# weidafeng/Efficient-SlowFast

Measured on AMD Instinct MI355X. Metric: clips/sec (8x8 224^2 SlowFast-R50+CMDA, train step fwd+bwd+allreduce+SGD), higher is better.
Workload: dtype f32

## Files before the change

### efficient-slowfast_amd/csrc/conv_bx.hip

```cpp
#include "bx.h"
#include <stdlib.h>

namespace {

constexpr int BXC_BM = 256;
constexpr int BXC_BK = 16;
constexpr int BXC_STAGES = 3;
constexpr int BXC_ROWB = BXC_BK * 2;
constexpr int BXC_A_STAGE = 3 * BXC_BM * BXC_ROWB;

struct BxArgs {
  sf_conv_desc d;
  const unsigned short* ap;
  const unsigned short* bp;
  float* ws;
  const float* scale;
  const float* bias;
  const float* res;
  float* out;
  int M, ntaps, cpk, nk, S, nk_per, nb_n, tiles;
  int tap_major;
  unsigned a_rows, a_bytes, b_bytes;
  unsigned a_plane, b_plane;
  unsigned wo_mul, wo_sh, ho_mul, ho_sh, to_mul, to_sh;
// ... 146 lines not shown
      cur_aso = (unsigned)l.c * (unsigned)BXC_ROWB;
    }
    const unsigned cur_bso = (unsigned)(l.tap * p.cpk + l.c) * (unsigned)BXC_ROWB;
    if constexpr (AF32) {
      __builtin_amdgcn_raw_ptr_buffer_load_lds(x_rs, (lds_void*)(smem + stage * STAGE + wave * 2048), 16, cur_f0, cur_aso,
                                               0, 0);
      __builtin_amdgcn_raw_ptr_buffer_load_lds(x_rs, (lds_void*)(smem + stage * STAGE + wave * 2048 + 1024), 16, cur_f1,
                                               cur_aso, 0, 0);
    } else {
      char* const sa = smem + stage * STAGE + wave * 1024;
#pragma unroll
      for (int g = 0; g < 3; ++g)
        __builtin_amdgcn_raw_ptr_buffer_load_lds(a_rs, (lds_void*)(sa + g * (BXC_BM * BXC_ROWB)), 16, cur_voff,
                                                 cur_aso + (unsigned)g * p.a_plane, 0, 0);
    }
    if (b_loader) {
      char* const sb = smem + stage * STAGE + A_ST + wave * 1024;
#pragma unroll
      for (int g = 0; g < 3; ++g)
        __builtin_amdgcn_raw_ptr_buffer_load_lds(b_rs, (lds_void*)(sb + g * (BN * BXC_ROWB)), 16, b_voff,
                                                 cur_bso + (unsigned)g * p.b_plane, 0, 0);
    }
    ls = next(l);
  };

  const unsigned frag_lane = (unsigned)(lane & 31) * BXC_ROWB + (unsigned)(((lane >> 5) ^ ((lane >> 4) & 1)) * 16);
  const unsigned a_frag = (unsigned)(wm * 64) * BXC_ROWB + frag_lane;
  const unsigned b_frag = A_ST + (unsigned)(wn * (BN / 2)) * BXC_ROWB + frag_lane;
  unsigned f_frag[2][2] = {{0, 0}, {0, 0}};
  if constexpr (AF32) {
#pragma unroll
    for (int i = 0; i < 2; ++i) {
      const int r = wm * 64 + i * 32 + (lane & 31);
#pragma unroll
      for (int q = 0; q < 2; ++q) f_frag[i][q] = (unsigned)r * 64u + (unsigned)(((2 * (lane >> 5) + q) ^ ((r >> 2) & 3)) * 16);
    }
  }

  f32x16 acc[2][NT];
#pragma unroll
  for (int i = 0; i < 2; ++i)
#pragma unroll
    for (int j = 0; j < NT; ++j)
#pragma unroll
      for (int e = 0; e < 16; ++e) acc[i][j][e] = 0.f;

  if (nsteps > 0) issue(0);
  if (nsteps > 1) issue(1);
  for (int it = 0; it < nsteps; ++it) {
    if (it + 1 < nsteps) {
      if constexpr (AF32) {
        if (b_loader) asm volatile("s_waitcnt vmcnt(5)" ::: "memory");
        else asm volatile("s_waitcnt vmcnt(2)" ::: "memory");
      } else {
        if (b_loader) asm volatile("s_waitcnt vmcnt(6)" ::: "memory");
        else asm volatile("s_waitcnt vmcnt(3)" ::: "memory");
      }
    } else {
      asm volatile("s_waitcnt vmcnt(0)" ::: "memory");
    }
    __builtin_amdgcn_s_barrier();
    if (it + 2 < nsteps) issue((it + 2) % BXC_STAGES);
    const char* const st = smem + (it % BXC_STAGES) * STAGE;
    u32x4 af[2][3], bf[NT][3];
    if constexpr (AF32) {
#pragma unroll
      for (int i = 0; i < 2; ++i) {
        const f32x4 lo = *reinterpret_cast<const f32x4*>(st + f_frag[i][0]);
        const f32x4 hi = *reinterpret_cast<const f32x4*>(st + f_frag[i][1]);
        split_pair(lo[0], lo[1], af[i], 0);
        split_pair(lo[2], lo[3], af[i], 1);
        split_pair(hi[0], hi[1], af[i], 2);
        split_pair(hi[2], hi[3], af[i], 3);
      }
    }
#pragma unroll
    for (int pc = 0; pc < 3; ++pc) {
      if constexpr (!AF32) {
#pragma unroll
        for (int i = 0; i < 2; ++i)
          af[i][pc] = *reinterpret_cast<const u32x4*>(st + a_frag + pc * (BXC_BM * BXC_ROWB) + i * (32 * BXC_ROWB));
      }
#pragma unroll
      for (int j = 0; j < NT; ++j)
        bf[j][pc] = *reinterpret_cast<const u32x4*>(st + b_frag + pc * (BN * BXC_ROWB) + j * (32 * BXC_ROWB));
    }
#pragma unroll
    for (int i = 0; i < 2; ++i)
#pragma unroll
      for (int j = 0; j < NT; ++j) acc[i][j] = mfma_split(af[i], bf[j], acc[i][j]);
  }

  const int col = lane & 31, rsub = 4 * (lane >> 5);
  if (DIRECT) {
#pragma unroll
    for (int j = 0; j < NT; ++j) {
      const int n = n0 + wn * (BN / 2) + j * 32 + col;
      const bool n_ok = n < d.Cout;
      const float sc = (p.scale && n_ok) ? p.scale[n] : 1.f;
      const float bi = (p.bias && n_ok) ? p.bias[n] : 0.f;
#pragma unroll
      for (int i = 0; i < 2; ++i) {
        float r[16];
#pragma unroll
        for (int e = 0; e < 16; ++e) {
          const int m = m0 + wm * 64 + i * 32 + (e & 3) + 8 * (e >> 2) + rsub;
          r[e] = (p.res && m < p.M && n_ok) ? p.res[(long)m * d.res_cs + d.res_coff + n] : 0.f;
        }
#pragma unroll
        for (int e = 0; e < 16; ++e) {
          const int m = m0 + wm * 64 + i * 32 + (e & 3) + 8 * (e >> 2) + rsub;
          if (m < p.M && n_ok) p.out[(long)m * d.out_cs + d.out_coff + n] = sf_act(acc[i][j][e] * sc + bi + r[e], d.act);
        }
      }
    }
    return;
  }
  float* const wsp = p.ws + (long)split * p.M * d.Cout;
#pragma unroll
  for (int i = 0; i < 2; ++i)
#pragma unroll
    for (int j = 0; j < NT; ++j) {
      const int n = n0 + wn * (BN / 2) + j * 32 + col;
#pragma unroll
      for (int e = 0; e < 16; ++e) {
        const int m = m0 + wm * 64 + i * 32 + (e & 3) + 8 * (e >> 2) + rsub;
        if (m < p.M && n < d.Cout) wsp[(long)m * d.Cout + n] = acc[i][j][e];
      }
    }
}

template <int BN>
__global__ __launch_bounds__(512, 4) void conv_pw_bx_kernel(const BxArgs p) {
  constexpr int A_STAGE = BXC_BM * 64;
  constexpr int B_STAGE = 3 * BN * BXC_ROWB;
  constexpr int STAGE = A_STAGE + B_STAGE;
  constexpr int NT = BN / 64;
  extern __shared__ __attribute__((aligned(16))) char smem[];
  const sf_conv_desc& d = p.d;
  const int tid = threadIdx.x, lane = tid & 63;
  const int wave = __builtin_amdgcn_readfirstlane(tid >> 6);
  const int wm = wave & 3, wn = wave >> 2;
  const int bid = xcd_remap(blockIdx.x, p.tiles);
  const int tile_m = bid / p.nb_n, tile_n = bid - tile_m * p.nb_n;
  const int m0 = tile_m * BXC_BM, n0 = tile_n * BN;
  const int nsteps = p.nk;

  const int lrow = lane >> 1;
  const unsigned lchunk = (unsigned)((lane & 1) ^ ((lrow >> 4) & 1)) * 16u;
  const bool b_loader = BN == 256 || wave < BN / 32;
  const int bn = n0 + 32 * wave + lrow;
  const unsigned kbytes = (unsigned)p.nk * (unsigned)BXC_ROWB;
  const unsigned b_voff = (unsigned)((b_loader && bn < d.Cout) ? bn : d.Cout) * kbytes + lchunk;
  const __amdgpu_buffer_rsrc_t b_rs = __builtin_amdgcn_make_buffer_rsrc((void*)p.bp, 0, p.b_bytes, 0x00020000);
  const __amdgpu_buffer_rsrc_t x_rs = __builtin_amdgcn_make_buffer_rsrc((void*)p.xf, 0, p.xf_bytes, 0x00020000);
  unsigned a_lvoff[2];
#pragma unroll
  for (int u = 0; u < 2; ++u) {
    const int r = 32 * wave + 16 * u + (lane >> 2);
    const int m = m0 + r;
    const unsigned chunk = (unsigned)((lane & 3) ^ ((r >> 2) & 3));
    a_lvoff[u] = m < p.M ? ((unsigned)m * (unsigned)d.in_cs + (unsigned)d.in_coff) * 4u + chunk * 16u : 0x80000000u;
  }
  auto issue = [&](int step) {
    char* const st = smem + (step % 2) * STAGE;
#pragma unroll
    for (int u = 0; u < 2; ++u)
      __builtin_amdgcn_raw_ptr_buffer_load_lds(x_rs, (lds_void*)(st + wave * 2048 + u * 1024), 16, a_lvoff[u],
                                               (unsigned)step * 64u, 0, 0);
    if (b_loader) {
      char* const sb = st + A_STAGE + wave * 1024;
#pragma unroll
      for (int g = 0; g < 3; ++g)
        __builtin_amdgcn_raw_ptr_buffer_load_lds(b_rs, (lds_void*)(sb + g * (BN * BXC_ROWB)), 16, b_voff,
                                                 (unsigned)step * (unsigned)BXC_ROWB + (unsigned)g * p.b_plane, 0, 0);
    }
  };
  unsigned a_frag[2][2];
#pragma unroll
  for (int i = 0; i < 2; ++i) {
    const int r = wm * 64 + i * 32 + (lane & 31);
#pragma unroll
    for (int q = 0; q < 2; ++q)
      a_frag[i][q] = (unsigned)r * 64u + (unsigned)(((2 * (lane >> 5) + q) ^ ((r >> 2) & 3)) * 16);
  }
  const unsigned frag_lane = (unsigned)(lane & 31) * BXC_ROWB + (unsigned)(((lane >> 5) ^ ((lane >> 4) & 1)) * 16);
  const unsigned b_frag = A_STAGE + (unsigned)(wn * (BN / 2)) * BXC_ROWB + frag_lane;

  f32x16 acc[2][NT];
#pragma unroll
  for (int i = 0; i < 2; ++i)
#pragma unroll
    for (int j = 0; j < NT; ++j)
#pragma unroll
      for (int e = 0; e < 16; ++e) acc[i][j][e] = 0.f;

  if (nsteps > 0) issue(0);
  for (int it = 0; it < nsteps; ++it) {
    asm volatile("s_waitcnt vmcnt(0)" ::: "memory");
    __builtin_amdgcn_s_barrier();
    if (it + 1 < nsteps) issue(it + 1);
    const char* const st = smem + (it % 2) * STAGE;
    u32x4 af[2][3], bf[NT][3];
#pragma unroll
    for (int i = 0; i < 2; ++i) {
      const f32x4 lo = *reinterpret_cast<const f32x4*>(st + a_frag[i][0]);
      const f32x4 hi = *reinterpret_cast<const f32x4*>(st + a_frag[i][1]);
      split_pair(lo[0], lo[1], af[i], 0);
      split_pair(lo[2], lo[3], af[i], 1);
      split_pair(hi[0], hi[1], af[i], 2);
      split_pair(hi[2], hi[3], af[i], 3);
    }
#pragma unroll
    for (int pc = 0; pc < 3; ++pc)
#pragma unroll
      for (int j = 0; j < NT; ++j)
        bf[j][pc] = *reinterpret_cast<const u32x4*>(st + b_frag + pc * (BN * BXC_ROWB) + j * (32 * BXC_ROWB));
#pragma unroll
    for (int i = 0; i < 2; ++i)
#pragma unroll
      for (int j = 0; j < NT; ++j) acc[i][j] = mfma_split(af[i], bf[j], acc[i][j]);
  }

  const int col = lane & 31, rsub = 4 * (lane >> 5);
  const bool want_stats = p.stats != nullptr;
  float* const kred = reinterpret_cast<float*>(smem);
  if (want_stats) __syncthreads();
#pragma unroll
  for (int j = 0; j < NT; ++j) {
    const int cl = wn * (BN / 2) + j * 32 + col;
    const int n = n0 + cl;
    const bool n_ok = n < d.Cout;
    const float sc = (p.scale && n_ok) ? p.scale[n] : 1.f;
    const float bi = (p.bias && n_ok) ? p.bias[n] : 0.f;
#pragma unroll
    for (int i = 0; i < 2; ++i) {
      float r[16];
#pragma unroll
      for (int e = 0; e < 16; ++e) {
        const int m = m0 + wm * 64 + i * 32 + (e & 3) + 8 * (e >> 2) + rsub;
        r[e] = (p.res && m < p.M && n_ok) ? p.res[(long)m * d.res_cs + d.res_coff + n] : 0.f;
      }
#pragma unroll
      for (int e = 0; e < 16; ++e) {
        const int m = m0 + wm * 64 + i * 32 + (e & 3) + 8 * (e >> 2) + rsub;
        const float v = sf_act(acc[i][j][e] * sc + bi + r[e], d.act);
        acc[i][j][e] = v;
        if (m < p.M && n_ok) p.out[(long)m * d.out_cs + d.out_coff + n] = v;
      }
    }
    if (want_stats && wm == 0 && rsub == 0) kred[cl] = acc[0][j][0];
  }
  if (!want_stats) return;
  __syncthreads();
  float* const sred = kred + BN;
#pragma unroll
  for (int j = 0; j < NT; ++j) {
    const int cl = wn * (BN / 2) + j * 32 + col;
    const float k0 = kred[cl];
    float s1 = 0.f, s2 = 0.f;
#pragma unroll
    for (int i = 0; i < 2; ++i)
#pragma unroll
      for (int e = 0; e < 16; ++e) {
        const int m = m0 + wm * 64 + i * 32 + (e & 3) + 8 * (e >> 2) + rsub;
        if (m < p.M) {
          const float dv = acc[i][j][e] - k0;
          s1 += dv;
          s2 += dv * dv;
        }
      }
    s1 += __shfl_xor(s1, 32, 64);
    s2 += __shfl_xor(s2, 32, 64);
    if (rsub == 0) {
      sred[(wm * BN + cl) * 2] = s1;
      sred[(wm * BN + cl) * 2 + 1] = s2;
    }
  }
  __syncthreads();
  if (tid < BN) {
    const int n = n0 + tid;
    if (n < d.Cout) {
      float s1 = 0.f, s2 = 0.f;
#pragma unroll
      for (int w = 0; w < 4; ++w) {
        s1 += sred[(w * BN + tid) * 2];
        s2 += sred[(w * BN + tid) * 2 + 1];
      }
      const int left = p.M - m0;
      const float cnt = (float)(left < BXC_BM ? left : BXC_BM);
      float* const o = p.stats + ((long)tile_m * (d.Cout >> 2) + (n >> 2)) * 16 + (n & 3);
      o[0] = cnt;
      o[4] = kred[tid];
      o[8] = s1;
      o[12] = s2;
    }
  }
}

struct BxwArgs {
  sf_conv_desc d;
  const unsigned short* xp;
  const unsigned short* zp;
  float* part;
  int M, Kc, S, chunk, nb_col, tiles;
  unsigned x_rows, x_plane, x_bytes, z_plane, z_bytes;
  unsigned wo_mul, wo_sh, ho_mul, ho_sh, to_mul, to_sh, ci_mul, ci_sh;
};

__device__ __forceinline__ u32x2 lds_tr(const char* p) {
  return lds_read_tr(reinterpret_cast<const unsigned short*>(p));
}
__device__ __forceinline__ u32x2 lds_tr_raw(unsigned lds_byte_addr) {
  u32x2 r;
  asm volatile("ds_read_b64_tr_b16 %0, %1" : "=v"(r) : "v"(lds_byte_addr));
  return r;
}

template <int BCO>
__global__ __launch_bounds__(512, 2) void conv_bx_wgrad_kernel(const BxwArgs p) {
  constexpr int BCOL = 256;
  constexpr int NWC = BCO == 256 ? 2 : 4;
  constexpr int NT = BCOL / NWC / 32;
  constexpr int ROW_A = BCO * 2, ROW_B = BCOL * 2;
  constexpr int PL_A = 16 * ROW_A, PL_B = 16 * ROW_B;
  constexpr int A_STAGE = 3 * PL_A, STAGE = A_STAGE + 3 * PL_B;
  constexpr int NA = PL_A / 1024;
  constexpr int CPR_A = BCO / 8;
  extern __shared__ __attribute__((aligned(16))) char smem[];
  const sf_conv_desc& d = p.d;
  const int tid = threadIdx.x, lane = tid & 63;
  const int wave = __builtin_amdgcn_readfirstlane(tid >> 6);
  const int wr = wave / NWC, wc = wave - wr * NWC;
  const int bid = xcd_remap(blockIdx.x, p.tiles * p.S);
  const int split = bid / p.tiles, tile = bid - split * p.tiles;
  const int tile_co = tile / p.nb_col, tile_col = tile - tile_co * p.nb_col;
  const int co0 = tile_co * BCO, col0 = tile_col * BCOL;
  const int mb = split * p.chunk;
  const int me = mb + p.chunk < p.M ? mb + p.chunk : p.M;
  const int nsteps = me > mb ? (me - mb + 15) / 16 : 0;

  const int b_pos = 2 * wave + (lane >> 5);
  const int b_cs = (lane & 31) ^ ((b_pos & 3) << 2);
  const int b_col = col0 + b_cs * 8;
  const bool b_colok = b_col < p.Kc;
  const unsigned b_tap = b_colok ? mdiv((unsigned)b_col, p.ci_mul, p.ci_sh) : 0u;
  const unsigned b_ci = b_colok ? (unsigned)b_col - b_tap * (unsigned)d.Cin : 0u;
  const int b_kw = (int)(b_tap % (unsigned)d.kW), b_kh = (int)((b_tap / (unsigned)d.kW) % (unsigned)d.kH),
            b_kt = (int)(b_tap / (unsigned)(d.kW * d.kH));
  const int b_dt = b_kt * d.dT - d.pT, b_dh = b_kh * d.dH - d.pH, b_dw = b_kw * d.dW - d.pW;
  const unsigned x_rowb = (unsigned)d.Cin * 2u;
  auto b_voff = [&](int m) -> unsigned {
    unsigned r = p.x_rows;
    if (m < me && b_colok) {
      const unsigned q1 = mdiv((unsigned)m, p.wo_mul, p.wo_sh);
      const int wo = (int)((unsigned)m - q1 * (unsigned)d.Wo);
      const unsigned q2 = mdiv(q1, p.ho_mul, p.ho_sh);
      const int ho = (int)(q1 - q2 * (unsigned)d.Ho);
      const unsigned q3 = mdiv(q2, p.to_mul, p.to_sh);
      const int to = (int)(q2 - q3 * (unsigned)d.To);
      const int ti = to * d.sT + b_dt, hi = ho * d.sH + b_dh, wi = wo * d.sW + b_dw;
      if ((unsigned)ti < (unsigned)d.Ti && (unsigned)hi < (unsigned)d.Hi && (unsigned)wi < (unsigned)d.Wi)
        r = (unsigned)((((int)q3 * d.Ti + ti) * d.Hi + hi) * d.Wi + wi);
    }
    return r * x_rowb + b_ci * 2u;
  };
  const bool a_loader = wave < NA;
  const int a_pos = wave * (64 / CPR_A) + lane / CPR_A;
  const int a_cs = (lane % CPR_A) ^ ((a_pos & 3) << 2);
  const int a_co = co0 + a_cs * 8;
  const unsigned z_rowb = (unsigned)d.Cout * 2u;
  auto a_voff = [&](int m) -> unsigned {
    const unsigned r = (m < me && a_co < d.Cout) ? (unsigned)m : (unsigned)p.M;
    return r * z_rowb + (unsigned)(a_co < d.Cout ? a_co : 0) * 2u;
  };
  const __amdgpu_buffer_rsrc_t x_rs = __builtin_amdgcn_make_buffer_rsrc((void*)p.xp, 0, p.x_bytes, 0x00020000);
  const __amdgpu_buffer_rsrc_t z_rs = __builtin_amdgcn_make_buffer_rsrc((void*)p.zp, 0, p.z_bytes, 0x00020000);
  int l_m = mb;
  auto issue = [&](int stage) {
    char* const st = smem + stage * STAGE;
    if (a_loader) {
      const unsigned vo = a_voff(l_m + a_pos);
#pragma unroll
      for (int pc = 0; pc < 3; ++pc)
        __builtin_amdgcn_raw_ptr_buffer_load_lds(z_rs, (lds_void*)(st + pc * PL_A + wave * 1024), 16, vo,
                                                 (unsigned)pc * p.z_plane, 0, 0);
    }
    const unsigned vb = b_voff(l_m + b_pos);
#pragma unroll
    for (int pc = 0; pc < 3; ++pc)
      __builtin_amdgcn_raw_ptr_buffer_load_lds(x_rs, (lds_void*)(st + A_STAGE + pc * PL_B + wave * 1024), 16, vb,
                                               (unsigned)pc * p.x_plane, 0, 0);
    l_m += 16;
  };

  const int g = lane >> 4, q = (lane & 15) >> 2, pq = lane & 3, h = g >> 1;
  unsigned a_addr[2], b_addr[NT];
#pragma unroll
  for (int i = 0; i < 2; ++i) {
    const int ch = wr * 64 + i * 32 + 16 * (g & 1) + 4 * pq;
    a_addr[i] = (unsigned)((8 * h + q) * ROW_A + (((ch >> 3) ^ (q << 2)) << 4) + (ch & 7) * 2);
  }
#pragma unroll
  for (int j = 0; j < NT; ++j) {
    const int ch = wc * (BCOL / NWC) + j * 32 + 16 * (g & 1) + 4 * pq;
    b_addr[j] = (unsigned)(A_STAGE + (8 * h + q) * ROW_B + (((ch >> 3) ^ (q << 2)) << 4) + (ch & 7) * 2);
  }

  f32x16 acc[2][NT];
#pragma unroll
  for (int i = 0; i < 2; ++i)
#pragma unroll
    for (int j = 0; j < NT; ++j)
#pragma unroll
      for (int e = 0; e < 16; ++e) acc[i][j][e] = 0.f;
  const unsigned lds_base = (unsigned)(uintptr_t)(__attribute__((address_space(3))) char*)smem;

  if (nsteps > 0) issue(0);
  if (nsteps > 1) issue(1);
  for (int it = 0; it < nsteps; ++it) {
    if (it + 1 < nsteps) {
      if (a_loader) asm volatile("s_waitcnt vmcnt(6)" ::: "memory");
      else asm volatile("s_waitcnt vmcnt(3)" ::: "memory");
    } else {
      asm volatile("s_waitcnt vmcnt(0)" ::: "memory");
    }
    __builtin_amdgcn_s_barrier();
    const unsigned st = lds_base + (unsigned)((it % BXC_STAGES) * STAGE);
    u32x4 af[2][3], bf[NT][3];
#pragma unroll
    for (int pc = 0; pc < 3; ++pc) {
#pragma unroll
      for (int i = 0; i < 2; ++i) {
        const u32x2 lo = lds_tr_raw(st + a_addr[i] + pc * PL_A), hi = lds_tr_raw(st + a_addr[i] + pc * PL_A + 4 * ROW_A);
        af[i][pc] = (u32x4){lo[0], lo[1], hi[0], hi[1]};
      }
#pragma unroll
      for (int j = 0; j < NT; ++j) {
        const u32x2 lo = lds_tr_raw(st + b_addr[j] + pc * PL_B), hi = lds_tr_raw(st + b_addr[j] + pc * PL_B + 4 * ROW_B);
        bf[j][pc] = (u32x4){lo[0], lo[1], hi[0], hi[1]};
      }
    }
    __builtin_amdgcn_sched_barrier(0);
    if (it + 2 < nsteps) issue((it + 2) % BXC_STAGES);
    __builtin_amdgcn_sched_barrier(0);
#pragma unroll
    for (int pc = 0; pc < 3; ++pc) {
      if constexpr (NT == 4)
        asm volatile("s_waitcnt lgkmcnt(0)"
                     : "+v"(af[0][pc]), "+v"(af[1][pc]), "+v"(bf[0][pc]), "+v"(bf[1][pc]), "+v"(bf[2][pc]), "+v"(bf[3][pc]));
      else
        asm volatile("s_waitcnt lgkmcnt(0)" : "+v"(af[0][pc]), "+v"(af[1][pc]), "+v"(bf[0][pc]), "+v"(bf[1][pc]));
    }
#pragma unroll
    for (int i = 0; i < 2; ++i)
#pragma unroll
      for (int j = 0; j < NT; ++j) acc[i][j] = mfma_split(af[i], bf[j], acc[i][j]);
  }

  float* const out = p.part + (long)split * d.Cout * p.Kc;
  const int ccol = lane & 31, rsub = 4 * (lane >> 5);
#pragma unroll
  for (int i = 0; i < 2; ++i)
#pragma unroll
    for (int j = 0; j < NT; ++j) {
      const int col = col0 + wc * (BCOL / NWC) + j * 32 + ccol;
#pragma unroll
      for (int e = 0; e < 16; ++e) {
        const int co = co0 + wr * 64 + i * 32 + (e & 3) + 8 * (e >> 2) + rsub;
        if (co < d.Cout && col < p.Kc) out[(long)co * p.Kc + col] = acc[i][j][e];
      }
    }
}

__global__ __launch_bounds__(256) void bx_split_rows_kernel(const float* __restrict__ x, int cs, int coff, long rows,
                                                            int C, unsigned short* __restrict__ planes) {
  const int c8 = C >> 3;
  const long total = (rows + 1) * c8;
  const long plane = (rows + 1) * (long)C;
  for (long idx = (long)blockIdx.x * 256 + threadIdx.x; idx < total; idx += (long)gridDim.x * 256) {
    const long r = idx / c8;
    const int c = (int)(idx - r * c8) * 8;
    u32x4 w[3];
    if (r < rows) {
      const f32x4 v0 = *reinterpret_cast<const f32x4*>(x + r * cs + coff + c);
      const f32x4 v1 = *reinterpret_cast<const f32x4*>(x + r * cs + coff + c + 4);
      split_pair(v0[0], v0[1], w, 0);
      split_pair(v0[2], v0[3], w, 1);
      split_pair(v1[0], v1[1], w, 2);
      split_pair(v1[2], v1[3], w, 3);
    } else {
      w[0] = w[1] = w[2] = (u32x4){0u, 0u, 0u, 0u};
    }
#pragma unroll
    for (int pc = 0; pc < 3; ++pc) *reinterpret_cast<u32x4*>(planes + pc * plane + r * C + c) = w[pc];
  }
}

struct BxSplitItem {
  const float* x;
  unsigned short* planes;
  long rows;
  int C, pad_;
};
__global__ __launch_bounds__(256) void bx_split_batched_kernel(const BxSplitItem* __restrict__ items,
                                                               const int* __restrict__ blk0, int n) {
  int lo = 0, hi = n;
  while (hi - lo > 1) {
    const int mid = (lo + hi) >> 1;
    if (blk0[mid] <= (int)blockIdx.x) lo = mid; else hi = mid;
  }
  const BxSplitItem it = items[lo];
  const int c8 = it.C >> 3;
  const long idx = (long)((int)blockIdx.x - blk0[lo]) * 256 + threadIdx.x;
  if (idx >= (it.rows + 1) * c8) return;
  const long plane = (it.rows + 1) * (long)it.C;
  const long r = idx / c8;
  const int c = (int)(idx - r * c8) * 8;
  u32x4 w[3];
  if (r < it.rows) {
    const f32x4 v0 = *reinterpret_cast<const f32x4*>(it.x + r * it.C + c);
    const f32x4 v1 = *reinterpret_cast<const f32x4*>(it.x + r * it.C + c + 4);
    split_pair(v0[0], v0[1], w, 0);
    split_pair(v0[2], v0[3], w, 1);
    split_pair(v1[0], v1[1], w, 2);
    split_pair(v1[2], v1[3], w, 3);
  } else {
    w[0] = w[1] = w[2] = (u32x4){0u, 0u, 0u, 0u};
  }
#pragma unroll
  for (int pc = 0; pc < 3; ++pc) *reinterpret_cast<u32x4*>(it.planes + pc * plane + r * it.C + c) = w[pc];
}

void magic(unsigned dv, unsigned* mul, unsigned* sh) {
  if (dv <= 1) { *mul = 0; *sh = 0; return; }
  unsigned l = 0;
  while ((1u << l) < dv) ++l;
  const unsigned long long num = 1ull << (31 + l);
  *mul = (unsigned)((num + dv - 1) / dv);
  *sh = l - 1;
}

int g_bx_enable = 1;

struct BxPlan { int bn, S, nk, nk_per, nb_n, tiles, direct; long a_rows; };

bool bx_af32(const sf_conv_desc* d);

bool bx_plan(const sf_conv_desc* d, BxPlan* pl, bool gate = true) {
  if (!g_bx_enable) return false;
  const long M = (long)d->N * d->To * d->Ho * d->Wo;
  const int ntaps = d->kT * d->kH * d->kW;
  if ((d->Cin % 16) || d->cin_pad != d->Cin || (d->in_cs % 4) || (d->in_coff % 4)) return false;
  if (d->Cout < 128 || (d->Cout % 4) || d->out_cmul != 1) return false;
  const int nk = ntaps * (d->Cin / BXC_BK);
  if (nk < 32 || M < 2048 || M > 0x7fffffffL) return false;
  if (d->transposed && (d->sT != 1 || d->sH != 1 || d->sW != 1)) return false;
  const long a_rows = (long)d->N * d->Ti * d->Hi * d->Wi;
  if (3 * (a_rows + 1) * d->Cin * 2 > 0xfffffff0L) return false;
  if (3L * (d->Cout + 1) * nk * BXC_ROWB > 0xfffffff0L) return false;
  pl->bn = d->Cout >= 256 ? 256 : 128;
  pl->nb_n = sf_cdiv(d->Cout, pl->bn);
  pl->tiles = sf_cdiv(M, BXC_BM) * pl->nb_n;
  pl->nk = nk;
  pl->a_rows = a_rows;
  const bool scatter = d->os_T > 1 || d->os_H > 1 || d->os_W > 1;
  const double step_us = pl->bn == 256 ? 2.05 : 1.6;
  const double out_mb = (double)M * d->Cout * 4e-6;
  int best = 1;
  double best_t = 1e30;
  for (int S = 1; S <= 16 && nk / S >= 8; ++S) {
    const long wg = (long)pl->tiles * S;
    if (wg > 2048) break;
    const long rounds = sf_cdiv(wg, 256);
    double t = 6.0 + (double)rounds * sf_cdiv(nk, S) * step_us;
    if (S > 1 || scatter) t += 3.0 + out_mb * (2.0 * S + 1.0) / 4.0;
    else t += out_mb / 4.0;
    if (t < best_t - 1e-9) { best_t = t; best = S; }
  }
  pl->S = best;
  pl->nk_per = sf_cdiv(nk, best);
  pl->direct = (best == 1 && !scatter) ? 1 : 0;
  if (gate && g_bx_enable < 2) {
    const double flop = 2.0 * M * (double)nk * BXC_BK * d->Cout;
    const double wave_us = flop / (nk >= 64 ? 100e6 : 90e6);
    const double split_us = bx_af32(d) ? 0.0 : 4.0 + (double)a_rows * d->Cin * 10e-6 / 3.0;
    const double pad = (double)(pl->nb_n * pl->bn) / (double)d->Cout;
    if (best_t * pad + split_us > 0.93 * wave_us) return false;
  }
  return true;
}


int g_pw_enable = 1;

struct PwPlan { int bn, nb_n, tiles, nk; };

bool pw_plan(const sf_conv_desc* d, PwPlan* pl, bool gate = true) {
  if (!g_bx_enable || !g_pw_enable) return false;
  if (d->kT != 1 || d->kH != 1 || d->kW != 1 || d->sT != 1 || d->sH != 1 || d->sW != 1 || d->pT || d->pH || d->pW)
    return false;
  if (d->To != d->Ti || d->Ho != d->Hi || d->Wo != d->Wi) return false;
  if (d->os_T > 1 || d->os_H > 1 || d->os_W > 1 || d->out_cmul != 1) return false;
  if ((d->Cin % 16) || d->cin_pad != d->Cin || (d->in_cs % 4) || (d->in_coff % 4)) return false;
  if (d->Cin < 64 || d->Cout < 64 || (d->Cout % 4)) return false;
  const long M = (long)d->N * d->To * d->Ho * d->Wo;
  if (M < 2048 || M > 0x3fffffffL) return false;
  if (((M - 1) * d->in_cs + d->in_coff + d->Cin) * 4L >= 0x7fffffffL) return false;
  pl->nk = d->Cin / BXC_BK;
  if (3L * (d->Cout + 1) * pl->nk * BXC_ROWB > 0xfffffff0L) return false;
  pl->bn = d->Cout <= 64 ? 64 : 128;
  pl->nb_n = sf_cdiv(d->Cout, pl->bn);
  pl->tiles = sf_cdiv(M, BXC_BM) * pl->nb_n;
  if (gate && g_pw_enable < 2 && g_bx_enable < 2) {
    const double mb = (double)M * (d->Cin + d->Cout) * 4e-6;
    if (pl->bn == 64) {
      if (d->Cin < 128) return false;
      return true;
    }
    if (d->Cout < 128) return false;
    double t_pw = 6.0 + (double)sf_cdiv(pl->tiles, 256) * pl->nk * 1.5;
    if (t_pw < mb / 4.5) t_pw = mb / 4.5;
    const double t_f32 = 6.0 + 2.0 * M * (double)d->Cin * d->Cout / 95e6 + 0.5 * mb / 4.5;
    if (t_pw > 0.85 * t_f32) return false;
  }
  return true;
}

template <int BN>
int launch_pw(const BxArgs& a, int grid, hipStream_t stream) {
  constexpr int lds = 2 * (BXC_BM * 64 + 3 * BN * BXC_ROWB);
  static_assert(lds >= (BN + 4 * BN * 2) * 4, "the statistics scratch lives in the stages");
  static SfLdsAttr at;
  if (!sf_ensure_dyn_lds(at, reinterpret_cast<const void*>(conv_pw_bx_kernel<BN>), lds)) return SF_ELAUNCH;
  hipLaunchKernelGGL((conv_pw_bx_kernel<BN>), dim3(grid), dim3(512), lds, stream, a);
  SF_CHECK_LAUNCH();
  return SF_OK;
}

bool bx_af32(const sf_conv_desc* d) {
  const long rows = (long)d->N * d->Ti * d->Hi * d->Wi;
  return ((rows - 1) * d->in_cs + d->in_coff + d->Cin) * 4L < 0x7fffffffL;
}

long align4(long floats) { return (floats + 3) & ~3L; }
long a_plane_floats(const sf_conv_desc* d, long a_rows) { return align4((3 * (a_rows + 1) * d->Cin + 1) / 2); }
long b_plane_floats(const sf_conv_desc* d, int nk) { return align4((3L * (d->Cout + 1) * nk * BXC_BK + 1) / 2); }

template <int BN, bool DIRECT, bool AF32>
int launch_bx_v(const BxArgs& a, int grid, hipStream_t stream) {
  constexpr int lds = BXC_STAGES * ((AF32 ? BXC_BM * 64 : BXC_A_STAGE) + 3 * BN * BXC_ROWB);
  static SfLdsAttr at;
  if (!sf_ensure_dyn_lds(at, reinterpret_cast<const void*>(conv_bx_kernel<BN, DIRECT, AF32>), lds)) return SF_ELAUNCH;
  hipLaunchKernelGGL((conv_bx_kernel<BN, DIRECT, AF32>), dim3(grid), dim3(512), lds, stream, a);
  SF_CHECK_LAUNCH();
  return SF_OK;
}

template <int BN, bool DIRECT>
int launch_bx(const BxArgs& a, int grid, hipStream_t stream) {
  if (a.xf) return launch_bx_v<BN, DIRECT, true>(a, grid, stream);
  return launch_bx_v<BN, DIRECT, false>(a, grid, stream);
}

}

int sf_conv_bx_tune(int value) { g_bx_enable = value; return SF_OK; }

int sf_conv_bx_takes(const sf_conv_desc* d) {
  BxPlan pl;
  return bx_plan(d, &pl) ? 1 : 0;
}

extern "C" long sf_bx_planes_elems(long rows, int C) { return 3 * (rows + 1) * (long)C; }

int sf_bx_split_rows(const float* x, int cs, int coff, long rows, int C, unsigned short* planes, hipStream_t s) {
  if ((C & 7) || (cs & 3) || (coff & 3) || !sf_aligned16(x) || !sf_aligned16(planes)) return SF_EALIGN;
  const long total = (rows + 1) * (C >> 3);
  long blocks = (total + 255) / 256;
  if (blocks > 256 * 16) blocks = 256 * 16;
  hipLaunchKernelGGL(bx_split_rows_kernel, dim3((unsigned)blocks), dim3(256), 0, s, x, cs, coff, rows, C, planes);
  SF_CHECK_LAUNCH();
  return SF_OK;
}

extern "C" int sf_bx_split(const float* x, int cs, int coff, long rows, int C, unsigned short* planes, void* stream) {
  if (!x || !planes || rows <= 0 || C <= 0) return SF_EINVAL;
  return sf_bx_split_rows(x, cs, coff, rows, C, planes, (hipStream_t)stream);
}

extern "C" int sf_bx_split_batched(const void* items, const int* blk0, int n, int nblocks, void* stream) {
  if (!items || !blk0 || n <= 0 || nblocks <= 0) return SF_EINVAL;
  hipLaunchKernelGGL(bx_split_batched_kernel, dim3(nblocks), dim3(256), 0, (hipStream_t)stream,
                     reinterpret_cast<const BxSplitItem*>(items), blk0, n);
  SF_CHECK_LAUNCH();
  return SF_OK;
}

int sf_conv_pw_tune(int value) { g_pw_enable = value; return SF_OK; }

int sf_conv_pw_takes(const sf_conv_desc* d) {
  PwPlan pl;
  return pw_plan(d, &pl) ? 1 : 0;
}

extern "C" long sf_conv_pw_ws_floats(const sf_conv_desc* d, int have_w_planes) {
  PwPlan pl;
  if (!d || !pw_plan(d, &pl)) return 0;
  return 4 + (have_w_planes ? 0 : b_plane_floats(d, pl.nk));
}

extern "C" long sf_conv_pw_stats_floats(const sf_conv_desc* d) {
  PwPlan pl;
  if (!d || d->transposed || d->act != SF_ACT_NONE || !pw_plan(d, &pl)) return 0;
  const long M = (long)d->N * d->To * d->Ho * d->Wo;
  return (long)sf_cdiv(M, BXC_BM) * 4 * d->Cout;
}

int sf_conv_pw_try(const sf_conv_desc* d, const float* in, const float* w_packed, const unsigned short* w_planes,
                   const float* scale, const float* bias, const float* res, float* out, float* ws, float* stats,
                   int* parts, hipStream_t stream) {
  PwPlan pl;
  if (parts) *parts = 0;
  if (!ws || !pw_plan(d, &pl)) return 1;
  if (!sf_aligned16(in) || !sf_aligned16(w_packed) || !sf_aligned16(ws)) return 1;
  if (w_planes && !sf_aligned16(w_planes)) return SF_EALIGN;
  if (stats && (scale || res || d->act != SF_ACT_NONE || !parts || !sf_aligned16(stats))) return 1;
  const long M = (long)d->N * d->To * d->Ho * d->Wo;
  if (!w_planes) {
    unsigned short* const bp = reinterpret_cast<unsigned short*>(ws + 4);
    const int rc = sf_bx_split_rows(w_packed, pl.nk * BXC_BK, 0, d->Cout, pl.nk * BXC_BK, bp, stream);
    if (rc != SF_OK) return rc;
    w_planes = bp;
  }
  BxArgs a = {};
  a.d = *d;
  a.bp = w_planes;
  a.scale = scale; a.bias = bias; a.res = res; a.out = out;
  a.M = (int)M;
  a.ntaps = 1; a.cpk = pl.nk; a.nk = pl.nk; a.S = 1; a.nk_per = pl.nk; a.nb_n = pl.nb_n; a.tiles = pl.tiles;
  a.b_plane = (unsigned)((long)(d->Cout + 1) * pl.nk * BXC_ROWB);
  a.b_bytes = 3u * a.b_plane;
  a.xf = in;
  a.xf_bytes = (unsigned)(((M - 1) * d->in_cs + d->in_coff + d->Cin) * 4L);
  a.stats = stats;
  if (stats) *parts = (int)sf_cdiv(M, BXC_BM);
  if (pl.bn == 64) return launch_pw<64>(a, pl.tiles, stream);
  return launch_pw<128>(a, pl.tiles, stream);
}

extern "C" int sf_conv_fwd_pw(const sf_conv_desc* d, const float* in, const float* w_packed,
                              const unsigned short* w_planes, const float* scale, const float* bias, const float* res,
                              float* out, float* ws, float* stats, int* parts, void* stream) {
  if (!d || !in || !w_packed || !out || !ws) return SF_EINVAL;
  const int rc = sf_conv_pw_try(d, in, w_packed, w_planes, scale, bias, res, out, ws, stats, parts, (hipStream_t)stream);
  return rc == 1 ? SF_ENOTTAKEN : rc;
}

extern "C" long sf_conv_bx_ws_floats(const sf_conv_desc* d, int have_in_planes, int have_w_planes) {
  BxPlan pl;
  if (!d || !bx_plan(d, &pl)) return 0;
  const long M = (long)d->N * d->To * d->Ho * d->Wo;
  return 4 + ((have_in_planes || bx_af32(d)) ? 0 : a_plane_floats(d, pl.a_rows)) +
         (have_w_planes ? 0 : b_plane_floats(d, pl.nk)) + (pl.direct ? 0 : (long)pl.S * M * d->Cout);
}

int sf_conv_splitk_finish(const sf_conv_desc* d, const float* ws, int S, const float* scale, const float* bias,
                          const float* res, float* out, hipStream_t s);

int sf_conv_bx_try(const sf_conv_desc* d, const float* in, const unsigned short* in_planes, const float* w_packed,
                   const unsigned short* w_planes, const float* scale, const float* bias, const float* res, float* out,
                   float* ws, hipStream_t stream) {
  BxPlan pl;
  if (!ws || !bx_plan(d, &pl)) return 1;
  if (!sf_aligned16(in) || !sf_aligned16(w_packed) || !sf_aligned16(ws)) return 1;
  if ((in_planes && !sf_aligned16(in_planes)) || (w_planes && !sf_aligned16(w_planes))) return SF_EALIGN;
  const long M = (long)d->N * d->To * d->Ho * d->Wo;
  float* cur = ws;
  int rc = SF_OK;
  const bool af32 = bx_af32(d);
  if (!in_planes && !af32) {
    unsigned short* const ap = reinterpret_cast<unsigned short*>(cur);
    cur += a_plane_floats(d, pl.a_rows);
    rc = sf_bx_split_rows(in, d->in_cs, d->in_coff, pl.a_rows, d->Cin, ap, stream);
    if (rc != SF_OK) return rc;
    in_planes = ap;
  }
  if (!w_planes) {
    unsigned short* const bp = reinterpret_cast<unsigned short*>(cur);
    cur += b_plane_floats(d, pl.nk);
    rc = sf_bx_split_rows(w_packed, pl.nk * BXC_BK, 0, d->Cout, pl.nk * BXC_BK, bp, stream);
    if (rc != SF_OK) return rc;
    w_planes = bp;
  }
  BxArgs a = {};
  a.d = *d;
  a.ap = in_planes; a.bp = w_planes; a.ws = cur;
  if (af32) {
    a.xf = in;
    a.xf_bytes = (unsigned)(((pl.a_rows - 1) * d->in_cs + d->in_coff + d->Cin) * 4L);
  }
  a.scale = scale; a.bias = bias; a.res = res; a.out = out;
  a.M = (int)M;
  a.ntaps = d->kT * d->kH * d->kW;
  a.cpk = d->Cin / BXC_BK;
  a.nk = pl.nk; a.S = pl.S; a.nk_per = pl.nk_per; a.nb_n = pl.nb_n; a.tiles = pl.tiles;
  a.tap_major = (d->sT > 1 || d->sH > 1 || d->sW > 1) ? 1 : 0;
  a.a_rows = (unsigned)pl.a_rows;
  a.a_plane = (unsigned)((pl.a_rows + 1) * d->Cin * 2);
  a.a_bytes = 3u * a.a_plane;
  a.b_plane = (unsigned)((long)(d->Cout + 1) * pl.nk * BXC_ROWB);
  a.b_bytes = 3u * a.b_plane;
  magic((unsigned)d->Wo, &a.wo_mul, &a.wo_sh);
  magic((unsigned)d->Ho, &a.ho_mul, &a.ho_sh);
  magic((unsigned)d->To, &a.to_mul, &a.to_sh);
  const int grid = pl.tiles * pl.S;
  if (pl.bn == 256) rc = pl.direct ? launch_bx<256, true>(a, grid, stream) : launch_bx<256, false>(a, grid, stream);
  else rc = pl.direct ? launch_bx<128, true>(a, grid, stream) : launch_bx<128, false>(a, grid, stream);
  if (rc != SF_OK) return rc;
  if (pl.direct) return SF_OK;
  return sf_conv_splitk_finish(d, cur, pl.S, scale, bias, res, out, stream);
}

extern "C" int sf_conv_fwd_bx(const sf_conv_desc* d, const float* in, const unsigned short* in_planes,
                              const float* w_packed, const unsigned short* w_planes, const float* scale,
                              const float* bias, const float* res, float* out, float* ws, void* stream) {
  if (!d || !in || !w_packed || !out || !ws) return SF_EINVAL;
  const int rc = sf_conv_bx_try(d, in, in_planes, w_packed, w_planes, scale, bias, res, out, ws, (hipStream_t)stream);
  return rc == 1 ? SF_ENOTTAKEN : rc;
}

namespace {

struct BxwPlan { int bco, S, nb_col, tiles; long chunk, x_rows; };

int g_bxw_enable = 1;

bool bxw_plan(const sf_conv_desc* d, BxwPlan* pl) {
  if (!g_bxw_enable) return false;
  const long M = (long)d->N * d->To * d->Ho * d->Wo;
  const int ntaps = d->kT * d->kH * d->kW;
  if ((d->Cin % 8) || d->cin_pad != d->Cin || (d->in_cs % 4) || (d->in_coff % 4)) return false;
  if (d->Cout < 128 || (d->Cout % 8)) return false;
  const long Kc = (long)ntaps * d->Cin;
  if (Kc < 512 || M < 2048 || M > 0x7ffffff0L) return false;
  const long x_rows = (long)d->N * d->Ti * d->Hi * d->Wi;
  if (3 * (x_rows + 1) * d->Cin * 2 > 0xfffffff0L || 3 * (M + 1) * d->Cout * 2 > 0xfffffff0L) return false;
  pl->bco = d->Cout >= 256 ? 256 : 128;
  pl->nb_col = sf_cdiv(Kc, 256);
  pl->tiles = sf_cdiv(d->Cout, pl->bco) * pl->nb_col;
  pl->x_rows = x_rows;
  const double step_us = pl->bco == 256 ? 2.0 : 1.1;
  const double out_mb = (double)d->Cout * Kc * 4e-6;
  int best = 1;
  double best_t = 1e30;
  const int maxS = (int)(M / 256 > 512 ? 512 : M / 256);
  for (int S = 1; S <= maxS; ++S) {
    const long wg = (long)pl->tiles * S;
    if (wg > 1536) break;
    const long rounds = sf_cdiv(wg, 256);
    const long steps = sf_cdiv(sf_cdiv(M, S), 16);
    const double t = 6.0 + (double)rounds * steps * step_us + out_mb * (2.0 * S + 1.0) / 4.0;
    if (t < best_t - 1e-9) { best_t = t; best = S; }
  }
  pl->S = best;
  pl->chunk = (sf_cdiv(M, best) + 15) / 16 * 16;
  if (g_bxw_enable < 2) {
    const double flop = 2.0 * M * (double)Kc * d->Cout;
    const double wave_us = flop / 95e6;
    const double split_us = 8.0 + ((double)x_rows * d->Cin + (double)M * d->Cout) * 10e-6 / 3.0;
    if (best_t + split_us > 0.93 * wave_us) return false;
  }
  return true;
}

long x_plane_floats(const sf_conv_desc* d, long x_rows) { return align4((3 * (x_rows + 1) * d->Cin + 1) / 2); }
long z_plane_floats(const sf_conv_desc* d, long M) { return align4((3 * (M + 1) * d->Cout + 1) / 2); }

template <int BCO>
int launch_bxw(const BxwArgs& a, int grid, hipStream_t stream) {
  constexpr int lds = BXC_STAGES * (3 * 16 * BCO * 2 + 3 * 16 * 256 * 2);
  static SfLdsAttr at;
  if (!sf_ensure_dyn_lds(at, reinterpret_cast<const void*>(conv_bx_wgrad_kernel<BCO>), lds)) return SF_ELAUNCH;
  hipLaunchKernelGGL((conv_bx_wgrad_kernel<BCO>), dim3(grid), dim3(512), lds, stream, a);
  SF_CHECK_LAUNCH();
  return SF_OK;
}

}

int sf_conv_bxw_tune(int value) { g_bxw_enable = value; return SF_OK; }

extern "C" int sf_conv_wgrad_bx_splits(const sf_conv_desc* d) {
  BxwPlan pl;
  return (d && bxw_plan(d, &pl)) ? pl.S : 0;
}

extern "C" long sf_conv_wgrad_bx_ws_floats(const sf_conv_desc* d, int have_x_planes, int have_dz_planes) {
  BxwPlan pl;
  if (!d || !bxw_plan(d, &pl)) return 0;
  const long M = (long)d->N * d->To * d->Ho * d->Wo;
  return 4 + (have_x_planes ? 0 : x_plane_floats(d, pl.x_rows)) + (have_dz_planes ? 0 : z_plane_floats(d, M));
}

extern "C" int sf_conv_wgrad_bx(const sf_conv_desc* d, const float* x, const unsigned short* x_planes, const float* dz,
                                int dz_cs, int dz_coff, const unsigned short* dz_planes, float* partial, float* ws,
                                void* stream) {
  BxwPlan pl;
  if (!d || !x || !dz || !partial || !ws) return SF_EINVAL;
  if (!bxw_plan(d, &pl)) return SF_ENOTTAKEN;
  if (!sf_aligned16(x) || !sf_aligned16(dz) || !sf_aligned16(ws) || !sf_aligned16(partial) || (dz_cs % 4) || (dz_coff % 4))
    return SF_EALIGN;
  hipStream_t s = (hipStream_t)stream;
  const long M = (long)d->N * d->To * d->Ho * d->Wo;
  float* cur = ws;
  int rc = SF_OK;
  if (!x_planes) {
    unsigned short* const xp = reinterpret_cast<unsigned short*>(cur);
    cur += x_plane_floats(d, pl.x_rows);
    rc = sf_bx_split_rows(x, d->in_cs, d->in_coff, pl.x_rows, d->Cin, xp, s);
    if (rc != SF_OK) return rc;
    x_planes = xp;
  }
  if (!dz_planes) {
    unsigned short* const zp = reinterpret_cast<unsigned short*>(cur);
    cur += z_plane_floats(d, M);
    rc = sf_bx_split_rows(dz, dz_cs, dz_coff, M, d->Cout, zp, s);
    if (rc != SF_OK) return rc;
    dz_planes = zp;
  }
  BxwArgs a;
  a.d = *d;
  a.xp = x_planes; a.zp = dz_planes; a.part = partial;
  a.M = (int)M;
  a.Kc = d->kT * d->kH * d->kW * d->Cin;
  a.S = pl.S; a.chunk = (int)pl.chunk; a.nb_col = pl.nb_col; a.tiles = pl.tiles;
  a.x_rows = (unsigned)pl.x_rows;
  a.x_plane = (unsigned)((pl.x_rows + 1) * d->Cin * 2);
  a.x_bytes = 3u * a.x_plane;
  a.z_plane = (unsigned)((M + 1) * d->Cout * 2);
  a.z_bytes = 3u * a.z_plane;
  magic((unsigned)d->Wo, &a.wo_mul, &a.wo_sh);
  magic((unsigned)d->Ho, &a.ho_mul, &a.ho_sh);
  magic((unsigned)d->To, &a.to_mul, &a.to_sh);
  magic((unsigned)d->Cin, &a.ci_mul, &a.ci_sh);
  const int grid = pl.tiles * pl.S;
  return pl.bco == 256 ? launch_bxw<256>(a, grid, s) : launch_bxw<128>(a, grid, s);
}
```

Baseline: 151.7.

## Fuse bf16x3 row split into wgrad kernel for 1x1 stride-1 convs

Adds a register-split variant of the split-bf16 wgrad kernel for pointwise, unstrided, unpadded convolutions. It reads x and dz directly as fp32 through buffer loads, splits each value into three bf16 planes in registers, and writes them to LDS inside the MMA loop with a 3-stage register pipeline. This skips the separate split_rows passes and their workspace round-trip. It also widens eligibility to small-Kc layers and drops the split overhead from the plan heuristic, which may route more layers here. The cost is extra VALU work and register pressure, plus BCO fixed at 128 for this path.

```diff
diff --git a/efficient-slowfast_amd/csrc/conv_bx.hip b/efficient-slowfast_amd/csrc/conv_bx.hip
--- a/efficient-slowfast_amd/csrc/conv_bx.hip
+++ b/efficient-slowfast_amd/csrc/conv_bx.hip
@@ -472,6 +472,9 @@
   sf_conv_desc d;
   const unsigned short* xp;
   const unsigned short* zp;
+  const float* xf;
+  const float* zf;
+  int z_cs, z_coff;
   float* part;
   int M, Kc, S, chunk, nb_col, tiles;
   unsigned x_rows, x_plane, x_bytes, z_plane, z_bytes;
@@ -487,7 +490,7 @@
   return r;
 }
 
-template <int BCO>
+template <int BCO, bool RS>
 __global__ __launch_bounds__(512, 2) void conv_bx_wgrad_kernel(const BxwArgs p) {
   constexpr int BCOL = 256;
   constexpr int NWC = BCO == 256 ? 2 : 4;
@@ -586,16 +589,7 @@
       for (int e = 0; e < 16; ++e) acc[i][j][e] = 0.f;
   const unsigned lds_base = (unsigned)(uintptr_t)(__attribute__((address_space(3))) char*)smem;
 
-  if (nsteps > 0) issue(0);
-  if (nsteps > 1) issue(1);
-  for (int it = 0; it < nsteps; ++it) {
-    if (it + 1 < nsteps) {
-      if (a_loader) asm volatile("s_waitcnt vmcnt(6)" ::: "memory");
-      else asm volatile("s_waitcnt vmcnt(3)" ::: "memory");
-    } else {
-      asm volatile("s_waitcnt vmcnt(0)" ::: "memory");
-    }
-    __builtin_amdgcn_s_barrier();
+  auto compute = [&](int it, auto&& ahead, auto&& during) {
     const unsigned st = lds_base + (unsigned)((it % BXC_STAGES) * STAGE);
     u32x4 af[2][3], bf[NT][3];
 #pragma unroll
@@ -612,7 +606,7 @@
       }
     }
     __builtin_amdgcn_sched_barrier(0);
-    if (it + 2 < nsteps) issue((it + 2) % BXC_STAGES);
+    ahead();
     __builtin_amdgcn_sched_barrier(0);
 #pragma unroll
     for (int pc = 0; pc < 3; ++pc) {
@@ -622,10 +616,87 @@
       else
         asm volatile("s_waitcnt lgkmcnt(0)" : "+v"(af[0][pc]), "+v"(af[1][pc]), "+v"(bf[0][pc]), "+v"(bf[1][pc]));
     }
+    during();
 #pragma unroll
     for (int i = 0; i < 2; ++i)
 #pragma unroll
       for (int j = 0; j < NT; ++j) acc[i][j] = mfma_split(af[i], bf[j], acc[i][j]);
+  };
+
+  if constexpr (!RS) {
+    if (nsteps > 0) issue(0);
+    if (nsteps > 1) issue(1);
+    for (int it = 0; it < nsteps; ++it) {
+      if (it + 1 < nsteps) {
+        if (a_loader) asm volatile("s_waitcnt vmcnt(6)" ::: "memory");
+        else asm volatile("s_waitcnt vmcnt(3)" ::: "memory");
+      } else {
+        asm volatile("s_waitcnt vmcnt(0)" ::: "memory");
+      }
+      __builtin_amdgcn_s_barrier();
+      compute(it, [&] { if (it + 2 < nsteps) issue((it + 2) % BXC_STAGES); }, [] {});
+    }
+  } else {
+    static_assert(BCO == 128, "register-split form: 4 dz channels per thread");
+    const int z_pos = 2 * wave + (lane >> 5), z_lc = (lane >> 1) & 15, z_half = lane & 1;
+    const int z_co = co0 + ((z_lc ^ ((z_pos & 3) << 2)) << 3) + 4 * z_half;
+    const bool z_colok = z_co < d.Cout;
+    const __amdgpu_buffer_rsrc_t xf_rs = __builtin_amdgcn_make_buffer_rsrc((void*)p.xf, 0, p.x_bytes, 0x00020000);
+    const __amdgpu_buffer_rsrc_t zf_rs = __builtin_amdgcn_make_buffer_rsrc((void*)p.zf, 0, p.z_bytes, 0x00020000);
+    const unsigned x_pitch = (unsigned)d.in_cs * 4u, z_pitch = (unsigned)p.z_cs * 4u;
+    const unsigned xb_off = (unsigned)(d.in_coff + b_col) * 4u, za_off = (unsigned)(p.z_coff + z_co) * 4u;
+    char* const b_dst = smem + A_STAGE + b_pos * ROW_B + (lane & 31) * 16;
+    char* const a_dst = smem + z_pos * ROW_A + z_lc * 16 + z_half * 8;
+    struct Regs { u32x4 b0, b1, a; };
+    auto load = [&](int k, Regs& r) {
+      const int m = mb + 16 * k + b_pos;
+      const unsigned ob = (b_colok && m < me) ? (unsigned)m * x_pitch + xb_off : p.x_bytes;
+      const unsigned oa = (z_colok && m < me) ? (unsigned)m * z_pitch + za_off : p.z_bytes;
+      r.b0 = __builtin_amdgcn_raw_buffer_load_b128(xf_rs, ob, 0, 0);
+      r.b1 = __builtin_amdgcn_raw_buffer_load_b128(xf_rs, ob + 16u, 0, 0);
+      r.a = __builtin_amdgcn_raw_buffer_load_b128(zf_rs, oa, 0, 0);
+    };
+    auto store = [&](int k, const Regs& r) {
+      const int so = (k % BXC_STAGES) * STAGE;
+      const f32x4 v0 = __builtin_bit_cast(f32x4, r.b0), v1 = __builtin_bit_cast(f32x4, r.b1);
+      const f32x4 va = __builtin_bit_cast(f32x4, r.a);
+      u32x4 w[3];
+      u32x2 wa[3];
+      split_pair(v0[0], v0[1], w, 0);
+      split_pair(v0[2], v0[3], w, 1);
+      split_pair(v1[0], v1[1], w, 2);
+      split_pair(v1[2], v1[3], w, 3);
+      split_pair(va[0], va[1], wa, 0);
+      split_pair(va[2], va[3], wa, 1);
+#pragma unroll
+      for (int pc = 0; pc < 3; ++pc) {
+        *reinterpret_cast<u32x4*>(b_dst + so + pc * PL_B) = w[pc];
+        *reinterpret_cast<u32x2*>(a_dst + so + pc * PL_A) = wa[pc];
+      }
+    };
+    auto interleave = [] {
+#pragma unroll
+      for (int i = 0; i < 2 * NT * 6; ++i) {
+        __builtin_amdgcn_sched_group_barrier(0x008, 1, 0);
+        __builtin_amdgcn_sched_group_barrier(0x002, 3, 0);
+      }
+    };
+    Regs r0, r1, r2;
+    load(0, r0);
+    load(1, r1);
+    load(2, r2);
+    store(0, r0);
+    auto step = [&](int it, Regs& next, const Regs& cur) {
+      asm volatile("s_waitcnt lgkmcnt(0)" ::: "memory");
+      __builtin_amdgcn_s_barrier();
+      compute(it, [&] { load(it + 3, next); }, [&] { store(it + 1, cur); });
+      interleave();
+    };
+    for (int it = 0; it < nsteps; it += 3) {
+      step(it, r0, r1);
+      step(it + 1, r1, r2);
+      step(it + 2, r2, r0);
+    }
   }
 
   float* const out = p.part + (long)split * d.Cout * p.Kc;
@@ -1002,7 +1073,7 @@
 
 namespace {
 
-struct BxwPlan { int bco, S, nb_col, tiles; long chunk, x_rows; };
+struct BxwPlan { int bco, S, nb_col, tiles, rs; long chunk, x_rows; };
 
 int g_bxw_enable = 1;
 
@@ -1013,14 +1084,17 @@
   if ((d->Cin % 8) || d->cin_pad != d->Cin || (d->in_cs % 4) || (d->in_coff % 4)) return false;
   if (d->Cout < 128 || (d->Cout % 8)) return false;
   const long Kc = (long)ntaps * d->Cin;
-  if (Kc < 512 || M < 2048 || M > 0x7ffffff0L) return false;
   const long x_rows = (long)d->N * d->Ti * d->Hi * d->Wi;
+  pl->rs = ntaps == 1 && d->sT == 1 && d->sH == 1 && d->sW == 1 && d->pT == 0 && d->pH == 0 && d->pW == 0 &&
+           x_rows == M && x_rows * d->in_cs * 4 <= 0xffffffc0L;
+  if (M > 0x7ffffff0L) return false;
+  if (pl->rs ? (M < 2048 && g_bxw_enable < 2) : (Kc < 512 || M < 2048)) return false;
   if (3 * (x_rows + 1) * d->Cin * 2 > 0xfffffff0L || 3 * (M + 1) * d->Cout * 2 > 0xfffffff0L) return false;
-  pl->bco = d->Cout >= 256 ? 256 : 128;
+  pl->bco = (d->Cout >= 256 && !pl->rs) ? 256 : 128;
   pl->nb_col = sf_cdiv(Kc, 256);
   pl->tiles = sf_cdiv(d->Cout, pl->bco) * pl->nb_col;
   pl->x_rows = x_rows;
-  const double step_us = pl->bco == 256 ? 2.0 : 1.1;
+  const double step_us = pl->bco == 256 ? 2.0 : pl->rs ? 1.3 : 1.1;
   const double out_mb = (double)d->Cout * Kc * 4e-6;
   int best = 1;
   double best_t = 1e30;
@@ -1029,16 +1103,16 @@
     const long wg = (long)pl->tiles * S;
     if (wg > 1536) break;
     const long rounds = sf_cdiv(wg, 256);
-    const long steps = sf_cdiv(sf_cdiv(M, S), 16);
+    const long steps = pl->rs ? sf_cdiv(sf_cdiv(M, S), 48) * 3 : sf_cdiv(sf_cdiv(M, S), 16);
     const double t = 6.0 + (double)rounds * steps * step_us + out_mb * (2.0 * S + 1.0) / 4.0;
     if (t < best_t - 1e-9) { best_t = t; best = S; }
   }
   pl->S = best;
-  pl->chunk = (sf_cdiv(M, best) + 15) / 16 * 16;
+  pl->chunk = pl->rs ? (sf_cdiv(M, best) + 47) / 48 * 48 : (sf_cdiv(M, best) + 15) / 16 * 16;
   if (g_bxw_enable < 2) {
     const double flop = 2.0 * M * (double)Kc * d->Cout;
     const double wave_us = flop / 95e6;
-    const double split_us = 8.0 + ((double)x_rows * d->Cin + (double)M * d->Cout) * 10e-6 / 3.0;
+    const double split_us = pl->rs ? 0.0 : 8.0 + ((double)x_rows * d->Cin + (double)M * d->Cout) * 10e-6 / 3.0;
     if (best_t + split_us > 0.93 * wave_us) return false;
   }
   return true;
@@ -1047,12 +1121,12 @@
 long x_plane_floats(const sf_conv_desc* d, long x_rows) { return align4((3 * (x_rows + 1) * d->Cin + 1) / 2); }
 long z_plane_floats(const sf_conv_desc* d, long M) { return align4((3 * (M + 1) * d->Cout + 1) / 2); }
 
-template <int BCO>
+template <int BCO, bool RS = false>
 int launch_bxw(const BxwArgs& a, int grid, hipStream_t stream) {
   constexpr int lds = BXC_STAGES * (3 * 16 * BCO * 2 + 3 * 16 * 256 * 2);
   static SfLdsAttr at;
-  if (!sf_ensure_dyn_lds(at, reinterpret_cast<const void*>(conv_bx_wgrad_kernel<BCO>), lds)) return SF_ELAUNCH;
-  hipLaunchKernelGGL((conv_bx_wgrad_kernel<BCO>), dim3(grid), dim3(512), lds, stream, a);
+  if (!sf_ensure_dyn_lds(at, reinterpret_cast<const void*>(conv_bx_wgrad_kernel<BCO, RS>), lds)) return SF_ELAUNCH;
+  hipLaunchKernelGGL((conv_bx_wgrad_kernel<BCO, RS>), dim3(grid), dim3(512), lds, stream, a);
   SF_CHECK_LAUNCH();
   return SF_OK;
 }
@@ -1070,6 +1144,7 @@
   BxwPlan pl;
   if (!d || !bxw_plan(d, &pl)) return 0;
   const long M = (long)d->N * d->To * d->Ho * d->Wo;
+  if (pl.rs && !have_x_planes && !have_dz_planes) return 4;
   return 4 + (have_x_planes ? 0 : x_plane_floats(d, pl.x_rows)) + (have_dz_planes ? 0 : z_plane_floats(d, M));
 }
 
@@ -1085,14 +1160,16 @@
   const long M = (long)d->N * d->To * d->Ho * d->Wo;
   float* cur = ws;
   int rc = SF_OK;
-  if (!x_planes) {
+  const bool rs = pl.rs && !x_planes && !dz_planes;
+  if (rs && M * dz_cs * 4 > 0xffffffc0L) return SF_ENOTTAKEN;
+  if (!rs && !x_planes) {
     unsigned short* const xp = reinterpret_cast<unsigned short*>(cur);
     cur += x_plane_floats(d, pl.x_rows);
     rc = sf_bx_split_rows(x, d->in_cs, d->in_coff, pl.x_rows, d->Cin, xp, s);
     if (rc != SF_OK) return rc;
     x_planes = xp;
   }
-  if (!dz_planes) {
+  if (!rs && !dz_planes) {
     unsigned short* const zp = reinterpret_cast<unsigned short*>(cur);
     cur += z_plane_floats(d, M);
     rc = sf_bx_split_rows(dz, dz_cs, dz_coff, M, d->Cout, zp, s);
@@ -1102,6 +1179,7 @@
   BxwArgs a;
   a.d = *d;
   a.xp = x_planes; a.zp = dz_planes; a.part = partial;
+  a.xf = x; a.zf = dz; a.z_cs = dz_cs; a.z_coff = dz_coff;
   a.M = (int)M;
   a.Kc = d->kT * d->kH * d->kW * d->Cin;
   a.S = pl.S; a.chunk = (int)pl.chunk; a.nb_col = pl.nb_col; a.tiles = pl.tiles;
@@ -1115,5 +1193,10 @@
   magic((unsigned)d->To, &a.to_mul, &a.to_sh);
   magic((unsigned)d->Cin, &a.ci_mul, &a.ci_sh);
   const int grid = pl.tiles * pl.S;
+  if (rs) {
+    a.x_bytes = (unsigned)(pl.x_rows * d->in_cs * 4);
+    a.z_bytes = (unsigned)(M * dz_cs * 4);
+    return launch_bxw<128, true>(a, grid, s);
+  }
   return pl.bco == 256 ? launch_bxw<256>(a, grid, s) : launch_bxw<128>(a, grid, s);
 }
```

Result: no change. 151.7, median of 2 (+0.0%).
